# psc0628/NeRF-PRV

Hardware: AMD Instinct MI355X
Metric: ray-samples/s (field evaluations composited; candidate views rendered + scored; scene baseline, field 256^3) (higher is better)
Workload: dtype f16

## Files before the change

### nerf_prv_amd/csrc/prv_kernels.hip

```cpp
#include "prv_kernels.hpp"

#include <algorithm>

#ifndef PRV_ABLATE
#define PRV_ABLATE 0
#endif

namespace prv {


__device__ __forceinline__ void morton16(uint32_t i, uint32_t& x, uint32_t& y) {
  x = (i & 1u) | ((i >> 1) & 2u) | ((i >> 2) & 4u) | ((i >> 3) & 8u);
  y = ((i >> 1) & 1u) | ((i >> 2) & 2u) | ((i >> 3) & 4u) | ((i >> 4) & 8u);
}

constexpr float kNgpDt = 1.7320508075688772f / 1024.0f;

__device__ __forceinline__ uint32_t march_ngp(const FieldDev& fd, const float o[3], const float d[3], float t0, float t1,
                                              uint32_t (*mw)[256], int& k_lo, int& k_hi, int& first_nz, int& last_nz) {
  const float dt = kNgpDt;
  first_nz = 32;
  last_nz = -1;
  k_lo = k_hi = 0;
  float ta = t0, tb = t1;
#pragma unroll
  for (int a = 0; a < 3; a++) {
    const float inv = 1.0f / d[a];
    const float u = (fd.occ_lo[a] - o[a]) * inv, w = (fd.occ_hi[a] - o[a]) * inv;
    ta = fmaxf(ta, fminf(u, w));
    tb = fminf(tb, fmaxf(u, w));
  }
  if (!(tb > ta)) return 0u;
  const float inv_dt = 1024.0f / 1.7320508075688772f;
  const int g_lo = max(0, (int)((ta - t0) * inv_dt) - 2);
  const int g_hi = min(kNgpMaxSteps, (int)((tb - t0) * inv_dt) + 3);
  if (g_lo >= g_hi) return 0u;
  k_lo = g_lo >> 5;
  k_hi = (g_hi + 31) >> 5;
  const bool coarse_ok = fd.occ_coarse != nullptr && 16.0f * dt <= 0.99f * 4.0f / (float)fd.occ_res;
  const int Rc_m1 = (fd.occ_res >> 2) - 1;
  const float fRc = (float)(fd.occ_res >> 2);
  const uint32_t Rc = (uint32_t)(Rc_m1 + 1);
  uint32_t n_live = 0u;
  for (int k = k_lo; k < k_hi; k++) {
    uint32_t w = 0u;
    bool pass = true;
    if (coarse_ok) {
      const float tm = fmaf((float)(32 * k + 16), dt, t0);
      const int cx = min(max((int)(fmaf(tm, d[0], o[0]) * fRc), 0), Rc_m1), cy = min(max((int)(fmaf(tm, d[1], o[1]) * fRc), 0), Rc_m1),
                cz = min(max((int)(fmaf(tm, d[2], o[2]) * fRc), 0), Rc_m1);
      const uint32_t bit = (uint32_t)cx + Rc * ((uint32_t)cy + Rc * (uint32_t)cz);
      pass = (fd.occ_coarse[bit >> 5] >> (bit & 31u)) & 1u;
    }
    if (pass) {
#pragma unroll
      for (int q0 = 0; q0 < 32; q0 += 8) {
        bool occ[8];
#pragma unroll
        for (int q = 0; q < 8; q++) {
          const int i = 32 * k + q0 + q;
          const float t = fmaf((float)i + 0.5f, dt, t0);
          occ[q] = occupied(fd, fmaf(t, d[0], o[0]), fmaf(t, d[1], o[1]), fmaf(t, d[2], o[2])) && t < t1;
        }
#pragma unroll
        for (int q = 0; q < 8; q++) w |= (uint32_t)occ[q] << (q0 + q);
      }
    }
    mw[k][threadIdx.x] = w;
    if (w != 0u) {
      if (first_nz == 32) first_nz = k;
      last_nz = k;
      n_live += (uint32_t)__popc(w);
    }
  }
  return n_live;
}


struct MarchRay {
  float o[3], d[3], t0, t1;
  uint32_t pix;
  bool valid, hit;
};

template <class PT>
__device__ __forceinline__ void march_ray_setup(const PT& P, const float occ_lo[3], const float occ_hi[3], uint32_t tx, uint32_t ty, MarchRay& r) {
  const uint32_t vi = blockIdx.y;
  uint32_t ix, iy, kk;
  if (P.spp_inner_log2 > 0) {
    kk = threadIdx.x & ((1u << P.spp_inner_log2) - 1u);
    morton16(threadIdx.x >> P.spp_inner_log2, ix, iy);
  } else {
    kk = blockIdx.z;
    morton16(threadIdx.x, ix, iy);
  }
  const int px = (int)((tx << P.tile_w_log2) + ix), py = (int)((ty << P.tile_h_log2) + iy);
  r.valid = px < P.W && py < P.H;
  r.pix = ((kk * gridDim.y + (uint32_t)vi) * (uint32_t)P.H + (uint32_t)py) * (uint32_t)P.W + (uint32_t)px;
  r.o[0] = r.o[1] = r.o[2] = 0.f;
  r.d[0] = r.d[1] = 0.f;
  r.d[2] = 1.f;
  r.t0 = r.t1 = 0.f;
  r.hit = false;
  bool maybe = r.valid;
  const CamDev& cam = P.cams[P.view_ids[vi]];
  float ox, oy;
  spp_offset((int)kk, ox, oy);
  if (cam.cull[2] > 0) {
    const int x0 = (int)(tx << P.tile_w_log2), y0 = (int)(ty << P.tile_h_log2);
    if (x0 + (1 << P.tile_w_log2) <= cam.cull[0] || x0 >= cam.cull[2] || y0 + (1 << P.tile_h_log2) <= cam.cull[1] || y0 >= cam.cull[3]) maybe = false;
  }
  if (maybe && !has_lens(cam)) {
    const float far = fmaxf(fmaxf(fabsf(cam.c2w[3] - 0.5f), fabsf(cam.c2w[7] - 0.5f)), fabsf(cam.c2w[11] - 0.5f));
    const float grow = fmaf(far, 1e-5f, 1e-3f);
    const float x = (((float)px + ox) - cam.cx) * __builtin_amdgcn_rcpf(cam.fx);
    const float y = (((float)py + oy) - cam.cy) * __builtin_amdgcn_rcpf(cam.fy);
    float ta = 0.0f, tb = __builtin_inff();
#pragma unroll
    for (int a = 0; a < 3; a++) {
      const float* mrow = cam.c2w + a * 4;
      const float inv = __builtin_amdgcn_rcpf(fmaf(mrow[0], x, fmaf(mrow[1], y, mrow[2])));
      const float u = ((occ_lo[a] - grow) - mrow[3]) * inv, w = ((occ_hi[a] + grow) - mrow[3]) * inv;
      ta = fmaxf(ta, fminf(u, w));
      tb = fminf(tb, fmaxf(u, w));
    }
    maybe = !(tb < ta);
  }
#if PRV_ABLATE & 8
  maybe = r.valid;
#endif
  if (maybe) {
    raygen(cam, px, py, ox, oy, r.o, r.d);
    r.hit = ray_aabb(r.o, r.d, r.t0, r.t1);
  }
}

struct MarchSink {
  void* queue;
  uint4* queue_ext;
  size_t ext_stride;
  uint32_t* queue_count;
  float* out_f32;
  uint32_t* out_u8;
};

template <bool NGP, bool WORDS_READY = false, bool IMAGE = true, class PT, class WordFn>
__device__ __forceinline__ void march_write(const PT& P, const MarchSink& Q, uint4 (*stage)[64 * kRecordWords], const MarchRay& r, bool live,
                                            unsigned long long b, uint32_t base, float dt, uint32_t m[4], int first_nz, int last_nz, WordFn word) {
  const int lane = threadIdx.x & 63;
  if (b != 0ull) {
    uint4* st = stage[threadIdx.x >> 6];
    if (live) {
      const uint32_t prefix = (uint32_t)__popcll(b & ((1ull << lane) - 1ull));
      uint4* rec = st + prefix * kRecordWords;
      uint32_t chunk_info = 1u << 16;
      if constexpr (NGP) {
        const int n_chunks = ((last_nz - first_nz) >> 2) + 1;
        chunk_info = (uint32_t)(32 * first_nz) | ((uint32_t)n_chunks << 16);
        if constexpr (!WORDS_READY) {
#pragma unroll
          for (int q = 0; q < 4; q++) m[q] = word(first_nz + q);
          uint4* ext = Q.queue_ext + (size_t)(base + prefix);
          for (int j = 1; j < ((PRV_ABLATE & 128) ? 1 : n_chunks); j++)
            ext[(size_t)(j - 1) * Q.ext_stride] = make_uint4(word(first_nz + 4 * j), word(first_nz + 4 * j + 1), word(first_nz + 4 * j + 2), word(first_nz + 4 * j + 3));
        }
      }
      rec[0] = make_uint4(__float_as_uint(r.o[0]), __float_as_uint(r.o[1]), __float_as_uint(r.o[2]), __float_as_uint(r.t0));
      rec[1] = make_uint4(__float_as_uint(r.d[0]), __float_as_uint(r.d[1]), __float_as_uint(r.d[2]), __float_as_uint(dt));
      rec[2] = make_uint4(m[0], m[1], m[2], m[3]);
      rec[3] = make_uint4(r.pix, chunk_info, 0u, 0u);
      reinterpret_cast<half8*>(rec)[4] = sh_fragment(0, r.d[0], r.d[1], r.d[2]);
      reinterpret_cast<half8*>(rec)[5] = sh_fragment(1, r.d[0], r.d[1], r.d[2]);
    }
    __builtin_amdgcn_fence(__ATOMIC_RELEASE, "wavefront");
    __builtin_amdgcn_wave_barrier();
    __builtin_amdgcn_fence(__ATOMIC_ACQUIRE, "wavefront");
    uint4* dst = reinterpret_cast<uint4*>(Q.queue) + (size_t)base * kRecordWords;
    const uint32_t n_words = (uint32_t)__popcll(b) * kRecordWords;
    for (uint32_t i = (uint32_t)lane; i < ((PRV_ABLATE & 256) ? 1u : n_words); i += 64u) dst[i] = st[i];
  }
  if constexpr (IMAGE) {
    if (!live && r.valid && !(PRV_ABLATE & 64)) {
      reinterpret_cast<float4*>(Q.out_f32)[r.pix] = make_float4(0.f, 0.f, 0.f, 0.f);
      if (P.last_pass && Q.out_u8) Q.out_u8[r.pix] = quantize_rgba8(0.f, 0.f, 0.f, 0.f, P.bg);
    }
  }
}

__device__ __forceinline__ uint32_t ray_octant(const float o[3], const float d[3], float t, const float lo[3], const float hi[3]) {
  uint32_t oct = 0u;
#pragma unroll
  for (int a = 0; a < 3; a++) oct |= (uint32_t)(fmaf(t, d[a], o[a]) > 0.5f * (lo[a] + hi[a])) << a;
  return oct;
}
__device__ __forceinline__ uint32_t region_reserve(uint32_t* queue_count, uint32_t n_seg, uint32_t seg_cap, uint32_t pref, uint32_t n) {
  for (uint32_t k = 0; k < n_seg; k++) {
    const uint32_t shard = (pref + k) % n_seg;
    uint32_t* c = queue_count + 16u * shard;
    if (k != 0u && __hip_atomic_load(c, __ATOMIC_RELAXED, __HIP_MEMORY_SCOPE_AGENT) >= seg_cap) continue;
    const uint32_t old = atomicAdd(c, n);
    if (old + n <= seg_cap) return shard * seg_cap + old;
    if (old < seg_cap) c[1] = seg_cap - old;
  }
  return 0u;
}

template <class PT>
__device__ __forceinline__ void march_count(const PT& P, uint32_t n_live) {
  uint32_t tot = n_live;
#pragma unroll
  for (int sh = 32; sh >= 1; sh >>= 1) tot += (uint32_t)__shfl_xor((int)tot, sh);
  const uint32_t sshard = (blockIdx.x + gridDim.x * (blockIdx.y + gridDim.y * blockIdx.z)) & 7u;
  if ((threadIdx.x & 63) == 0 && tot) atomicAdd(P.stat + 8u * (1u + sshard), (unsigned long long)tot);
}

template <bool NGP, bool IMAGE = true, class PT, class WordFn>
__device__ __forceinline__ void march_emit(const PT& P, const MarchSink& Q, uint4 (*stage)[64 * kRecordWords], const MarchRay& r, bool live,
                                           uint32_t n_live, float dt, uint32_t m[4], int first_nz, int last_nz, WordFn word) {
  const unsigned long long b = __ballot(live);
  const int lane = threadIdx.x & 63;
  uint32_t base = 0;
  if (b != 0ull) {
    if (lane == (int)__builtin_ctzll(b)) {
      uint32_t i0 = 0u;
      if constexpr (NGP) {
        i0 = 32u * (uint32_t)first_nz + (uint32_t)__builtin_ctz(word(first_nz));
        if (P.spatial_regions != 2) i0 = (i0 + 32u * (uint32_t)last_nz + 31u - (uint32_t)__builtin_clz(word(last_nz))) >> 1;
      } else {
        i0 = m[0] ? (uint32_t)__builtin_ctz(m[0]) : m[1] ? 32u + (uint32_t)__builtin_ctz(m[1]) : m[2] ? 64u + (uint32_t)__builtin_ctz(m[2]) : 96u + (uint32_t)__builtin_ctz(m[3]);
        if (P.spatial_regions != 2) {
          const uint32_t i1 = m[3] ? 127u - (uint32_t)__builtin_clz(m[3]) : m[2] ? 95u - (uint32_t)__builtin_clz(m[2]) : m[1] ? 63u - (uint32_t)__builtin_clz(m[1]) : 31u - (uint32_t)__builtin_clz(m[0]);
          i0 = (i0 + i1) >> 1;
        }
      }
      const uint32_t lin = blockIdx.x + gridDim.x * (blockIdx.y + gridDim.y * blockIdx.z);
      const uint32_t pref = P.spatial_regions ? ray_octant(r.o, r.d, fmaf((float)i0 + 0.5f, dt, r.t0), P.field.occ_lo, P.field.occ_hi) * (uint32_t)P.n_sub + lin % (uint32_t)P.n_sub
                                              : lin;
      base = region_reserve(Q.queue_count, (uint32_t)P.n_seg, P.seg_cap, pref % (uint32_t)P.n_seg, (uint32_t)__popcll(b));
    }
    base = __shfl(base, (int)__builtin_ctzll(b));
  }
  march_write<NGP, false, IMAGE>(P, Q, stage, r, live, b, base, dt, m, first_nz, last_nz, word);
  if (b != 0ull) march_count(P, n_live);
}

template <bool NGP, bool IMAGE>
__device__ __forceinline__ void march_compact_body(MarchParams P) {
  __shared__ uint4 stage[4][64 * kRecordWords];
  __shared__ uint32_t mw[NGP ? 32 : 1][256];
  const uint32_t vi = blockIdx.y;
  uint32_t tx, ty;
  if (P.live_grid) {
    const CamDev& cv = P.cams[P.view_ids[vi]];
    uint32_t tx0 = 0, ty0 = 0, tx1 = P.tiles_x, ty1 = P.tiles_y;
    if (cv.cull[2] > 0) {
      tx0 = (uint32_t)cv.cull[0] >> P.tile_w_log2;
      ty0 = (uint32_t)cv.cull[1] >> P.tile_h_log2;
      tx1 = min(P.tiles_x, ((uint32_t)cv.cull[2] + (1u << P.tile_w_log2) - 1u) >> P.tile_w_log2);
      ty1 = min(P.tiles_y, ((uint32_t)max(cv.cull[3], 0) + (1u << P.tile_h_log2) - 1u) >> P.tile_h_log2);
    }
    const uint32_t w = tx1 > tx0 ? tx1 - tx0 : 0u, h = ty1 > ty0 ? ty1 - ty0 : 0u;
    if (blockIdx.x >= w * h) return;
    ty = ty0 + blockIdx.x / w;
    tx = tx0 + blockIdx.x - (blockIdx.x / w) * w;
  } else {
    ty = blockIdx.x / P.tiles_x;
    tx = blockIdx.x - ty * P.tiles_x;
  }
  MarchRay r;
  march_ray_setup(P, P.field.occ_lo, P.field.occ_hi, tx, ty, r);
  const float* o = r.o;
  const float* d = r.d;
  const float t0 = r.t0, t1 = r.t1;
  float dt = 0.f;
  uint32_t m[4] = {0, 0, 0, 0};
  uint32_t n_live = 0u;
  int k_lo = 0, k_hi = 0, first_nz = 32, last_nz = -1;
  bool live = false;
#if PRV_ABLATE & 32
  r.hit = false;
#endif
  if (r.hit) {
#if PRV_ABLATE & 16
    live = (t0 + t1 + d[0] + o[1]) == 1.0e30f;
#else
    if constexpr (NGP) {
      dt = kNgpDt;
      n_live = march_ngp(P.field, o, d, t0, t1, mw, k_lo, k_hi, first_nz, last_nz);
      live = first_nz < 32;
    } else {
      dt = (t1 - t0) / (float)P.S;
      const bool coarse_ok = P.field.occ_coarse != nullptr && 1.5f * dt <= 0.99f * 4.0f / (float)P.field.occ_res;
      int g_lo = 0, g_hi = P.S;
      {
        float ta = t0, tb = t1;
#pragma unroll
        for (int a = 0; a < 3; a++) {
          const float inv = 1.0f / d[a];
          const float u = (P.field.occ_lo[a] - o[a]) * inv, w = (P.field.occ_hi[a] - o[a]) * inv;
          ta = fmaxf(ta, fminf(u, w));
          tb = fminf(tb, fmaxf(u, w));
        }
        if (!(tb > ta)) {
          g_hi = 0;
        } else if (dt > 0.0f) {
          const float inv_dt = __builtin_amdgcn_rcpf(dt);
          g_lo = max(0, (int)((ta - t0) * inv_dt) - 2) & ~3;
          g_hi = min(P.S, (int)((tb - t0) * inv_dt) + 3);
        }
      }
      const int Rc_m1 = (P.field.occ_res >> 2) - 1;
      const float fRc = (float)(P.field.occ_res >> 2);
      const float ocx = o[0] * fRc, ocy = o[1] * fRc, ocz = o[2] * fRc, dcx = d[0] * fRc, dcy = d[1] * fRc, dcz = d[2] * fRc;
      const uint32_t Rc = (uint32_t)(Rc_m1 + 1);
#pragma unroll
      for (int k = 0; k < 4; k++) {
        uint32_t w = 0u;
        const int lo = max(g_lo, 32 * k), hi = min(g_hi, 32 * k + 32);
        if (lo < hi) {
          uint32_t pass = 0xffu;
          if (coarse_ok) {
            pass = 0u;
#pragma unroll
            for (int j = 0; j < 8; j++) {
              const int g = 32 * k + 4 * j;
// ... 146 lines not shown
    for (int e = 0; e < E; e++) {
      first_any = min(first_any, first_nz[e]);
      last_any = max(last_any, last_nz[e]);
    }
    const unsigned long long b_any = __ballot(first_any < 32);
    uint32_t pref = blockIdx.x + gridDim.x * (blockIdx.y + gridDim.y * blockIdx.z);
    if (P.spatial_regions && b_any != 0ull) {
      const uint32_t oct = ray_octant(o, d, fmaf((float)(16 * (min(first_any, 31) + last_any)) + 16.0f, dt, t0), P.occ_lo, P.occ_hi);
      pref = (uint32_t)__shfl((int)oct, (int)__builtin_ctzll(b_any)) * (uint32_t)P.n_sub + pref % (uint32_t)P.n_sub;
    }
    const uint32_t shard = pref % (uint32_t)P.n_seg;
    uint32_t* qc = nullptr;
    uint32_t mine = 0u, tot = 0u;
#pragma unroll
    for (int e = 0; e < E; e++) {
      b[e] = __ballot(first_nz[e] < 32);
      if (lane == e) {
        qc = P.mem[e].queue_count;
        mine = (uint32_t)__popcll(b[e]);
      }
      tot += n_live[e];
    }
    uint32_t got = 0u;
    if (mine) got = region_reserve(qc, (uint32_t)P.n_seg, P.seg_cap, shard, mine);
#pragma unroll
    for (int e = 0; e < E; e++) base[e] = __shfl(got, e);
    march_count(P, tot);
  }
  uint32_t m[E][4];
#pragma unroll
  for (int e = 0; e < E; e++)
#pragma unroll
    for (int q = 0; q < 4; q++) m[e][q] = 0u;
  {
    int k2_lo = 32, k2_hi = -1;
#pragma unroll
    for (int e = 0; e < E; e++) {
      k2_lo = min(k2_lo, first_nz[e]);
      k2_hi = max(k2_hi, last_nz[e]);
    }
    uint32_t acc[E][4];
#pragma unroll
    for (int e = 0; e < E; e++)
#pragma unroll
      for (int q = 0; q < 4; q++) acc[e][q] = 0u;
    for (int k = k2_lo; k <= k2_hi; k++) {
      uint32_t w[E];
      bool behind = false;
#pragma unroll
      for (int e = 0; e < E; e++) behind = behind || (k - first_nz[e] >= kWin && k <= last_nz[e]);
      if (!((passmask >> k) & 1u)) {
#pragma unroll
        for (int e = 0; e < E; e++) w[e] = 0u;
      } else if (behind) {
        fine_word(k, w);
      } else {
#pragma unroll
        for (int e = 0; e < E; e++) {
          const int j = k - first_nz[e];
          w[e] = (j >= 0 && k <= last_nz[e]) ? mw[e][j][threadIdx.x] : 0u;
        }
      }
#pragma unroll
      for (int e = 0; e < E; e++) {
        const int j = k - first_nz[e];
        if (j < 0 || k > last_nz[e]) continue;
        const int q = j & 3;
        if (j < 4) {
#pragma unroll
          for (int u = 0; u < 4; u++)
            if (q == u) m[e][u] = w[e];
        } else {
#pragma unroll
          for (int u = 0; u < 4; u++)
            if (q == u) acc[e][u] = w[e];
          if ((q == 3 || k == last_nz[e]) && !(PRV_ABLATE & 128)) {
            const uint32_t slot = base[e] + (uint32_t)__popcll(b[e] & ((1ull << lane) - 1ull));
            P.mem[e].queue_ext[(size_t)((j >> 2) - 1) * ext_stride + slot] = make_uint4(acc[e][0], acc[e][1], acc[e][2], acc[e][3]);
#pragma unroll
            for (int u = 0; u < 4; u++) acc[e][u] = 0u;
          }
        }
      }
    }
  }
#pragma unroll
  for (int e = 0; e < E; e++) {
    const MarchSink Q{P.mem[e].queue, P.mem[e].queue_ext, ext_stride, P.mem[e].queue_count, P.mem[e].out_f32, P.mem[e].out_u8};
    march_write<true, true>(P, Q, stage, r, first_nz[e] < 32, b[e], base[e], dt, m[e], first_nz[e], last_nz[e], [](int) { return 0u; });
  }
}

__global__ __launch_bounds__(256) void occ_interleave_kernel(OccInterleaveParams P) {
  const uint32_t c = blockIdx.x * 256u + threadIdx.x;
  if (c >= P.n_cells) return;
  uint32_t v = 0u;
  for (int e = 0; e < P.n_members; e++) v |= ((P.bits[e][c >> 5] >> (c & 31u)) & 1u) << e;
  P.out[c] = (uint8_t)v;
}


__device__ __forceinline__ void clock_stamp_begin(unsigned long long* stat) {
  if (blockIdx.x == 0 && threadIdx.x == 0) {
    stat[4] = __builtin_readcyclecounter();
    stat[5] = __builtin_amdgcn_s_memrealtime();
  }
}
__device__ __forceinline__ void clock_stamp_end(unsigned long long* stat) {
  if (blockIdx.x == 0 && threadIdx.x == 0) {
    atomicAdd(stat + 2, __builtin_readcyclecounter() - stat[4]);
    atomicAdd(stat + 3, __builtin_amdgcn_s_memrealtime() - stat[5]);
  }
}

__device__ __forceinline__ int lane_id() { return (int)(threadIdx.x & 63u); }

__device__ __forceinline__ float entropy_add(float p, float H) { return p >= 1.17549435e-38f ? fmaf(p, -__builtin_amdgcn_logf(p), H) : H; }

template <int F, int NDENSE, bool NGP, bool CACHE, int MODE>
__device__ __forceinline__ void render_queue64_body(RenderParams P, const RenderPlanesParams* X) {
  constexpr bool FOOT = MODE == kRenderFootprint, SURF = MODE == kRenderSurface;
  constexpr bool DEPTH = MODE == kRenderDepth || FOOT, ENTROPY = MODE == kRenderEntropy || FOOT || SURF;
  constexpr bool DSTATE = DEPTH || SURF;
  constexpr int kDWord = ENTROPY ? 4 : 6;
  constexpr int kMoveWords = (ENTROPY ? 4 : 6) + (DSTATE ? 1 : 0);
  constexpr int kFrags = ENTROPY ? 8 : kNumFrags;
  __shared__ half8 wl[kFrags * 64];
  __shared__ uint32_t mv[4][32][kMoveWords];
  constexpr uint32_t kPoolCap = 192;
  __shared__ uint32_t pool[kPoolCap][kMoveWords];
  __shared__ uint32_t pool_n, pool_lock;
  for (int i = threadIdx.x; i < kFrags * 64; i += 256) wl[i] = P.field.frags64[i];
  if (threadIdx.x == 0) {
    pool_n = 0u;
    pool_lock = 0u;
  }
  __syncthreads();
  auto pool_acquire = [&]() {
    if (lane_id() == 0)
      while (atomicCAS(&pool_lock, 0u, 1u) != 0u) __builtin_amdgcn_s_sleep(2);
    __builtin_amdgcn_fence(__ATOMIC_ACQUIRE, "workgroup");
    __builtin_amdgcn_wave_barrier();
  };
  auto pool_release = [&]() {
    __builtin_amdgcn_fence(__ATOMIC_RELEASE, "workgroup");
    __builtin_amdgcn_wave_barrier();
    if (lane_id() == 0) atomicExch(&pool_lock, 0u);
  };
  const LevelDev* __restrict__ lvl = P.field.levels;
  const HashConsts hc = {P.field.hash_my_b, P.field.hash_mz_b, P.field.hash_m_b, (uint32_t)P.field.wide_offsets};

  const int lane = threadIdx.x & 63, r = lane & 31, g = lane >> 5;

  bool active = false;
  uint32_t pix = 0, rec_i = 0;
  float o[3] = {0, 0, 0}, d[3] = {0, 0, 1}, t0 = 0.f, dt = 0.f;
  uint32_t cur = 0, m1 = 0, m2 = 0, m3 = 0, base = 0;
  float T = 1.f, cr = 0.f, cg = 0.f, cb = 0.f;
  float D = 0.f;
  float Hs = 0.f;
  half8 shA = {0, 0, 0, 0, 0, 0, 0, 0}, shB = {0, 0, 0, 0, 0, 0, 0, 0};
  bool drained = false;
  unsigned long long n_eval = 0ull, n_rounds = 0ull;
  constexpr int kCached = CACHE ? 32 / F - NDENSE : 1;
  CornerCache<F> cc[kCached];
#pragma unroll
  for (int j = 0; j < kCached; j++) cc[j].key = ~0u;
  clock_stamp_begin(P.stat_evaluated);
  uint32_t q_cur = 0, q_end = 0;
  const uint32_t n_seg = (uint32_t)P.n_segments;
  const uint32_t n_sub = (uint32_t)max(P.n_sub, 1);
  uint32_t seg = n_seg > 1u ? (((uint32_t)__builtin_amdgcn_s_getreg((3 << 11) | 20) & 7u) % (n_seg / n_sub)) * n_sub + (blockIdx.x * 4u + (threadIdx.x >> 6)) % n_sub : 0u;
  uint32_t seg_tried = 0;
  const uint4* __restrict__ queue = reinterpret_cast<const uint4*>(P.queue);

  auto take_ray = [&](uint32_t ri, uint32_t next) {
    const uint4* rec = queue + (size_t)ri * kRecordWords;
    const uint4 q0 = rec[0], q1 = rec[1], q3 = rec[3];
    uint4 mk = rec[2];
    o[0] = __uint_as_float(q0.x); o[1] = __uint_as_float(q0.y); o[2] = __uint_as_float(q0.z);
    t0 = __uint_as_float(q0.w);
    d[0] = __uint_as_float(q1.x); d[1] = __uint_as_float(q1.y); d[2] = __uint_as_float(q1.z);
    dt = __uint_as_float(q1.w);
    pix = q3.x;
    rec_i = ri;
    base = 0u;
    if constexpr (NGP) {
      const uint32_t base0 = q3.y & 0xffffu;
      base = base0;
      if (next >= base0 + 128u) {
        const uint32_t j = (next - base0) >> 7;
        mk = P.queue_ext[(size_t)(j - 1u) * ((size_t)P.seg_cap * (size_t)P.n_segments) + (size_t)ri];
        base = base0 + 128u * j;
      }
    }
    cur = mk.x; m1 = mk.y; m2 = mk.z; m3 = mk.w;
    while (base + 32u <= next) {
      cur = m1; m1 = m2; m2 = m3; m3 = 0u;
      base += 32u;
    }
    if (next > base) cur &= ~0u << (next & 31u);
    while (cur == 0u && (m1 | m2 | m3) != 0u) {
      cur = m1; m1 = m2; m2 = m3; m3 = 0u;
      base += 32u;
    }
    active = true;
  };
  auto next_chunk = [&]() -> bool {
    const uint32_t info = queue[(size_t)rec_i * kRecordWords + 3].y;
    const uint32_t base0 = info & 0xffffu, n_chunks = info >> 16;
    for (uint32_t j = ((base - base0) >> 7) + 1u; j < n_chunks; j++) {
      const uint4 mk = P.queue_ext[(size_t)(j - 1u) * ((size_t)P.seg_cap * (size_t)P.n_segments) + (size_t)rec_i];
      if ((mk.x | mk.y | mk.z | mk.w) == 0u) continue;
      cur = mk.x; m1 = mk.y; m2 = mk.z; m3 = mk.w;
      base = base0 + 128u * j;
      while (cur == 0u) {
        cur = m1; m1 = m2; m2 = m3; m3 = 0u;
        base += 32u;
      }
      return true;
    }
    return false;
  };

  for (;;) {
    const bool relocate = (n_rounds & 6ull) == 0ull;
    if (relocate && !drained && P.merge_max > 0) {
      const unsigned long long act0 = __ballot(active);
      const uint32_t aA = (uint32_t)act0, aB = (uint32_t)(act0 >> 32);
      const uint32_t nA = (uint32_t)__popc(aA), nB = (uint32_t)__popc(aB);
      int src = -1;
      if (nA != 0u && nB != 0u) {
        if (nA <= (uint32_t)P.merge_max && nA <= 32u - nB) src = 0;
        else if (nB <= (uint32_t)P.merge_max && nB <= 32u - nA) src = 1;
      }
      if (src >= 0) {
        const uint32_t a_src = src == 0 ? aA : aB, a_dst = src == 0 ? aB : aA, n_src = src == 0 ? nA : nB;
        const uint32_t below = (1u << r) - 1u;
        uint32_t(*slot)[kMoveWords] = mv[threadIdx.x >> 6];
        if (g == src && active) {
          uint32_t* e = slot[__popc(a_src & below)];
          e[0] = rec_i;
          e[1] = base + (uint32_t)__builtin_ctz(cur);
          e[2] = __float_as_uint(T);
          if constexpr (ENTROPY) {
            e[3] = __float_as_uint(Hs);
          } else {
            e[3] = __float_as_uint(cr);
            e[4] = __float_as_uint(cg);
            e[5] = __float_as_uint(cb);
          }
          if constexpr (DSTATE) e[kDWord] = __float_as_uint(D);
          active = false;
        }
        __builtin_amdgcn_fence(__ATOMIC_RELEASE, "wavefront");
        __builtin_amdgcn_wave_barrier();
        __builtin_amdgcn_fence(__ATOMIC_ACQUIRE, "wavefront");
        const uint32_t kth = (uint32_t)__popc(~a_dst & below);
        if (!((a_dst >> r) & 1u) && kth < n_src) {
          const uint32_t* e = slot[kth];
          const uint32_t ri = e[0];
          if constexpr (!ENTROPY) {
            const half8 sh = reinterpret_cast<const half8*>(queue + (size_t)ri * kRecordWords)[4 + g];
            if (src == 0) shB = sh;
            else shA = sh;
          }
          if (g != src) {
            T = __uint_as_float(e[2]);
            if constexpr (ENTROPY) {
              Hs = __uint_as_float(e[3]);
            } else {
              cr = __uint_as_float(e[3]); cg = __uint_as_float(e[4]); cb = __uint_as_float(e[5]);
            }
            if constexpr (DSTATE) D = __uint_as_float(e[kDWord]);
            take_ray(ri, e[1]);
          }
        }
        __builtin_amdgcn_wave_barrier();
      }
    }
    if (P.pool_on && (relocate || drained)) {
      const unsigned long long act1 = __ballot(active);
      const uint32_t below = (1u << r) - 1u;
      const uint32_t in_pool = *(volatile uint32_t*)&pool_n;
#pragma unroll
      for (int grp = 0; grp < 2; grp++) {
        const uint32_t a_g = grp == 0 ? (uint32_t)act1 : (uint32_t)(act1 >> 32), n_g = (uint32_t)__popc(a_g);
        if (!drained && n_g != 0u && n_g <= (uint32_t)P.merge_max && in_pool + n_g <= kPoolCap) {
          pool_acquire();
          const uint32_t at = *(volatile uint32_t*)&pool_n;
          const bool fits = at + n_g <= kPoolCap;
          if (fits && g == grp && active) {
            uint32_t* e = pool[at + (uint32_t)__popc(a_g & below)];
            e[0] = rec_i;
            e[1] = base + (uint32_t)__builtin_ctz(cur);
            e[2] = __float_as_uint(T);
            if constexpr (ENTROPY) {
              e[3] = __float_as_uint(Hs);
            } else {
              e[3] = __float_as_uint(cr);
              e[4] = __float_as_uint(cg);
              e[5] = __float_as_uint(cb);
            }
            if constexpr (DSTATE) e[kDWord] = __float_as_uint(D);
            active = false;
          }
          if (fits && lane == 0) *(volatile uint32_t*)&pool_n = at + n_g;
          pool_release();
        }
      }
      const unsigned long long act2 = __ballot(active);
#pragma unroll
      for (int grp = 0; grp < 2; grp++) {
        const uint32_t a_g = grp == 0 ? (uint32_t)act2 : (uint32_t)(act2 >> 32);
        const uint32_t n_idle = 32u - (uint32_t)__popc(a_g);
        if (n_idle == 0u || (a_g == 0u && !drained) || *(volatile uint32_t*)&pool_n == 0u) continue;
        pool_acquire();
        const uint32_t have = *(volatile uint32_t*)&pool_n;
        const uint32_t take = min(have, n_idle), from = have - take;
        const uint32_t kth = (uint32_t)__popc(~a_g & below);
        uint32_t ent[kMoveWords] = {};
        const bool mine = !((a_g >> r) & 1u) && kth < take;
        if (mine) {
#pragma unroll
          for (int q = 0; q < kMoveWords; q++) ent[q] = pool[from + kth][q];
        }
        if (lane == 0) *(volatile uint32_t*)&pool_n = from;
        pool_release();
        if (mine) {
          if constexpr (!ENTROPY) {
            const half8 sh = reinterpret_cast<const half8*>(queue + (size_t)ent[0] * kRecordWords)[4 + g];
            if (grp == 0) shA = sh;
            else shB = sh;
          }
          if (g == grp) {
            T = __uint_as_float(ent[2]);
            if constexpr (ENTROPY) {
              Hs = __uint_as_float(ent[3]);
            } else {
              cr = __uint_as_float(ent[3]); cg = __uint_as_float(ent[4]); cb = __uint_as_float(ent[5]);
            }
            if constexpr (DSTATE) D = __uint_as_float(ent[kDWord]);
            take_ray(ent[0], ent[1]);
          }
        }
      }
    }
    const unsigned long long idle = __ballot(!active);
    const bool needA = (uint32_t)idle == 0xffffffffu, needB = (uint32_t)(idle >> 32) == 0xffffffffu;
    if (!drained && (needA || needB)) {
#pragma unroll
      for (int grp = 0; grp < 2; grp++) {
        if (!(grp == 0 ? needA : needB)) continue;
        while (q_cur == q_end && !drained) {
          uint32_t claim = 0;
          if (lane == 0) claim = atomicAdd(P.queue_head + 16u * seg, kClaim);
          claim = __builtin_amdgcn_readfirstlane(claim);
          const uint32_t s_lo = seg * P.seg_cap, s_cnt = min(P.queue_count[16u * seg], P.seg_cap) - P.queue_count[16u * seg + 1u];
          if (claim < s_cnt) {
            q_cur = s_lo + claim;
            q_end = min(q_cur + kClaim, s_lo + s_cnt);
          } else if (++seg_tried >= n_seg) {
            drained = true;
          } else {
            seg = seg + 1u == n_seg ? 0u : seg + 1u;
          }
        }
        const uint32_t avail = min(32u, q_end - q_cur);
        if ((uint32_t)r < avail) {
          if constexpr (!ENTROPY) {
            const half8 sh = reinterpret_cast<const half8*>(queue + (size_t)(q_cur + (uint32_t)r) * kRecordWords)[4 + g];
            if (grp == 0) shA = sh;
            else shB = sh;
          }
          if (g == grp) {
            T = 1.f; cr = 0.f; cg = 0.f; cb = 0.f;
            if constexpr (DSTATE) D = 0.f;
            if constexpr (ENTROPY) Hs = 0.f;
            take_ray(q_cur + (uint32_t)r, 0u);
          }
        }
        q_cur += avail;
      }
    }
    const unsigned long long act = __ballot(active);
    if (act == 0ull) {
      if (drained && (!P.pool_on || *(volatile uint32_t*)&pool_n == 0u)) break;
      continue;
    }
    n_eval += (unsigned long long)__popcll(act);
    n_rounds += 2ull;

    half8 f[4];
#pragma unroll
    for (int s = 0; s < 4; s++) asm volatile("" : "=v"(f[s]));
    bool last = false;
    float ts = 0.f;
    if (active) {
      const uint32_t i = base + (uint32_t)__builtin_ctz(cur);
      cur &= cur - 1u;
      if (cur == 0u) {
        last = (m1 | m2 | m3) == 0u;
        while (cur == 0u && !last) {
          cur = m1; m1 = m2; m2 = m3; m3 = 0u;
          base += 32u;
        }
        if constexpr (NGP) {
          if (last) last = !next_chunk();
        }
      }
      const float t = fmaf((float)i + 0.5f, dt, t0);
      if constexpr (DSTATE) ts = t;
      encode_sample<F, NDENSE, CACHE>(P.field.table, lvl, hc, fmaf(t, d[0], o[0]), fmaf(t, d[1], o[1]), fmaf(t, d[2], o[2]), f, cc);
    }
    swap_halves(f[0], f[1]);
    swap_halves(f[2], f[3]);
    const half8 fA[2] = {f[0], f[2]}, fB[2] = {f[1], f[3]};
    MlpOut2 mo;
    if constexpr (ENTROPY) mlp_density2(wl, lane, fA, fB, mo.densA, mo.densB);
    else mo = mlp_forward2(wl, lane, fA, fB, shA, shB);
    const float dens = g ? mo.densB[8] : mo.densA[0];
    float lr = 0.f, lg = 0.f, lb = 0.f;
    if constexpr (!ENTROPY) {
      lr = g ? mo.rgbB[8] : mo.rgbA[0];
      lg = g ? mo.rgbB[9] : mo.rgbA[1];
      lb = g ? mo.rgbB[10] : mo.rgbA[2];
    }

    bool done = false;
    if (active) {
      const float sigma = fast_exp(dens + P.field.density_bias);
      const float alpha = 1.0f - fast_exp(-(sigma * dt));
      const float wgt = alpha * T;
      if constexpr (ENTROPY) {
        Hs = entropy_add(wgt, Hs);
      } else {
        cr = fmaf(wgt, fast_sigmoid(lr), cr);
        cg = fmaf(wgt, fast_sigmoid(lg), cg);
        cb = fmaf(wgt, fast_sigmoid(lb), cb);
      }
      if constexpr (DEPTH) D = fmaf(wgt, ts, D);
      T = T * (1.0f - alpha);
      if constexpr (SURF) {
        if (D == 0.f && T <= X->T_cross) D = ts;
      }
      done = last || T < P.min_T;
    }
    if (done) {
      if constexpr (!ENTROPY) {
        const float4 v = make_float4(cr, cg, cb, 1.0f - T);
        reinterpret_cast<float4*>(P.out_f32)[pix] = v;
        if (P.last_pass && P.out_u8) P.out_u8[pix] = quantize_rgba8(v.x, v.y, v.z, v.w, P.bg);
      }
      if constexpr (ENTROPY) {
        X->out_entropy[pix] = entropy_add(T, Hs);
        X->out_alpha[pix] = 1.0f - T;
      }
      if constexpr (DSTATE) {
        const CamDev& cam = X->cams[X->view_ids[(pix / X->npix) % X->nb]];
        const float fx = cam.c2w[2], fy = cam.c2w[6], fz = cam.c2w[10];
        const float inv = 1.0f / sqrtf(fmaf(fx, fx, fmaf(fy, fy, fz * fz)));
        X->out_depth[pix] = D * (fmaf(d[0], fx, fmaf(d[1], fy, d[2] * fz)) * inv);
        if constexpr (SURF) X->out_hit[pix] = D > 0.f ? 1.0f : 0.0f;
      }
      active = false;
    }
  }
  if (lane == 0 && n_eval) {
    atomicAdd(P.stat_evaluated, n_eval);
    atomicAdd(P.stat_evaluated + 1, n_rounds);
  }
  clock_stamp_end(P.stat_evaluated);
}

template <int F, int NDENSE, bool NGP, bool CACHE = false>
__global__ __launch_bounds__(256)
__attribute__((amdgpu_waves_per_eu(CACHE ? 2 : NDENSE == 0 ? 1 : 3)))
void render_queue64_kernel(RenderParams P) {
  render_queue64_body<F, NDENSE, NGP, CACHE, kRenderColour>(P, nullptr);
}

template <int F, int NDENSE, bool NGP, int MODE>
__global__ __launch_bounds__(256)
__attribute__((amdgpu_waves_per_eu(NDENSE == 0 ? 1 : MODE == kRenderSurface && F == 4 && !NGP ? 4 : 3)))
void render_planes_kernel(RenderPlanesParams P) {
  render_queue64_body<F, NDENSE, NGP, false, MODE>(P.r, &P);
}

__device__ __forceinline__ int32_t first_hit_dda(const FieldDev& fd, const float o[3], const float d[3], float max_range) {
  float t0, t1;
  int32_t result = -1;
  if (ray_aabb(o, d, t0, t1)) {
    if (t1 > max_range) t1 = max_range;
    if (t1 > t0) {
      const int R = fd.occ_res;
      const float fR = (float)R;
      const float ts = t0 + 1e-6f;
      int c[3], step[3];
      float tmax[3], tdelta[3];
#pragma unroll
      for (int a = 0; a < 3; a++) {
        const float p = clamp01(fmaf(ts, d[a], o[a])) * fR;
        c[a] = min((int)p, R - 1);
        if (d[a] > 0.f) {
          step[a] = 1;
          tmax[a] = (((float)(c[a] + 1)) / fR - o[a]) / d[a];
          tdelta[a] = 1.0f / (fR * d[a]);
        } else if (d[a] < 0.f) {
          step[a] = -1;
          tmax[a] = (((float)c[a]) / fR - o[a]) / d[a];
          tdelta[a] = -1.0f / (fR * d[a]);
        } else {
          step[a] = 0;
          tmax[a] = __builtin_inff();
          tdelta[a] = __builtin_inff();
        }
      }
      for (;;) {
        const uint32_t bit = (uint32_t)c[0] + (uint32_t)R * ((uint32_t)c[1] + (uint32_t)R * (uint32_t)c[2]);
        if ((fd.occ[bit >> 5] >> (bit & 31)) & 1u) {
          result = (int32_t)bit;
          break;
        }
        const int a = tmax[0] < tmax[1] ? (tmax[0] < tmax[2] ? 0 : 2) : (tmax[1] < tmax[2] ? 1 : 2);
        const float tm = a == 0 ? tmax[0] : (a == 1 ? tmax[1] : tmax[2]);
        if (tm > t1) break;
        if (a == 0) { c[0] += step[0]; tmax[0] += tdelta[0]; if (c[0] < 0 || c[0] >= R) break; }
        else if (a == 1) { c[1] += step[1]; tmax[1] += tdelta[1]; if (c[1] < 0 || c[1] >= R) break; }
        else { c[2] += step[2]; tmax[2] += tdelta[2]; if (c[2] < 0 || c[2] >= R) break; }
      }
    }
  }
  return result;
}

__global__ __launch_bounds__(256) void first_hit_kernel(FieldDev fd, const CamDev* __restrict__ cams, int W, int H,
                                                        float max_range, int32_t* __restrict__ out) {
  const int i = blockIdx.x * 256 + threadIdx.x;
  if (i >= W * H) return;
  const int v = blockIdx.y;
  const int px = i % W, py = i / W;
  float o[3], d[3], t0, t1;
  raygen(cams[v], px, py, 0.5f, 0.5f, o, d);
  (void)t0;
  (void)t1;
  const int32_t result = first_hit_dda(fd, o, d, max_range);
  out[(size_t)v * W * H + i] = result;
}

__global__ __launch_bounds__(256) void precept_kernel(FieldDev fd, const float* __restrict__ voxels, int n, PreceptPose pose,
                                                      Rs2Intr in, float max_range, int32_t* __restrict__ out) {
  const int i = blockIdx.x * 256 + threadIdx.x;
  if (i >= n) return;
  const float origin[3] = {(float)pose.c2w[3], (float)pose.c2w[7], (float)pose.c2w[11]};
  double v[3];
#pragma unroll
  for (int r = 0; r < 3; r++)
    v[r] = pose.w2c[r * 4] * (double)voxels[i * 3] + pose.w2c[r * 4 + 1] * (double)voxels[i * 3 + 1] +
           pose.w2c[r * 4 + 2] * (double)voxels[i * 3 + 2] + pose.w2c[r * 4 + 3];
  const float point_3d[3] = {(float)v[0], (float)v[1], (float)v[2]};
  float pixel[2];
  rs2_project(pixel, in, point_3d);
  int32_t result = -1;
  if (!(pixel[0] < 0 || pixel[0] > (float)in.width || pixel[1] < 0 || pixel[1] > (float)in.height)) {
    const float ipx[2] = {(float)(int)pixel[0], (float)(int)pixel[1]};
    float pt[3], d[3];
    rs2_deproject(pt, in, ipx, 1.0f);
#pragma unroll
    for (int r = 0; r < 3; r++) {
      const float e = (float)(pose.c2w[r * 4] * (double)pt[0] + pose.c2w[r * 4 + 1] * (double)pt[1] +
                              pose.c2w[r * 4 + 2] * (double)pt[2] + pose.c2w[r * 4 + 3]);
      d[r] = e - origin[r];
    }
    const float n2 = fmaf(d[0], d[0], fmaf(d[1], d[1], d[2] * d[2]));
    const float inv = 1.0f / sqrtf(n2);
#pragma unroll
    for (int r = 0; r < 3; r++) d[r] = d[r] * inv;
    result = first_hit_dda(fd, origin, d, max_range);
  }
  out[i] = result;
}

__global__ __launch_bounds__(256) void spp_reduce_kernel(const float4* __restrict__ stage, size_t n, int spp, float inv_spp,
                                                         float b0, float b1, float b2, float b3,
                                                         float4* __restrict__ out, uint32_t* __restrict__ out_u8) {
  const float bg[4] = {b0, b1, b2, b3};
  for (size_t i = (size_t)blockIdx.x * 256 + threadIdx.x; i < n; i += (size_t)gridDim.x * 256) {
    float4 a = stage[i];
    for (int k = 1; k < spp; k++) {
      const float4 v = stage[(size_t)k * n + i];
      a.x = a.x + v.x; a.y = a.y + v.y; a.z = a.z + v.z; a.w = a.w + v.w;
    }
    a.x *= inv_spp; a.y *= inv_spp; a.z *= inv_spp; a.w *= inv_spp;
    out[i] = a;
    if (out_u8) out_u8[i] = quantize_rgba8(a.x, a.y, a.z, a.w, bg);
  }
}

__global__ __launch_bounds__(256) void spp_reduce_depth_kernel(const float* __restrict__ stage, size_t n, int spp, float inv_spp,
                                                               float* __restrict__ out) {
  for (size_t i = (size_t)blockIdx.x * 256 + threadIdx.x; i < n; i += (size_t)gridDim.x * 256) {
    float a = stage[i];
    for (int k = 1; k < spp; k++) a = a + stage[(size_t)k * n + i];
    out[i] = a * inv_spp;
  }
}


__global__ __launch_bounds__(256) void quantize_kernel(const float4* __restrict__ in, size_t n,
                                                       float b0, float b1, float b2, float b3,
                                                       uint32_t* __restrict__ out) {
  const float bg[4] = {b0, b1, b2, b3};
  for (size_t i = (size_t)blockIdx.x * 256 + threadIdx.x; i < n; i += (size_t)gridDim.x * 256) {
    float4 v = in[i];
    out[i] = quantize_rgba8(v.x, v.y, v.z, v.w, bg);
  }
}


// ... 644 lines not shown
```

### nerf_prv_amd/csrc/prv_kernels.hpp

```cpp
#pragma once
#include "../../include/prv.h"
#include "prv_device.hpp"
#include <type_traits>

namespace prv {

constexpr size_t kRecordBytes = 96;
constexpr int kRecordWords = 6;
constexpr uint32_t kClaim = 64;
constexpr int kMaxSamples = 128;
constexpr int kNgpMaxSteps = PRV_NGP_MAX_STEPS;
constexpr int kExtChunks = kNgpMaxSteps / 128 - 1;
constexpr size_t kExtBytes = (size_t)kExtChunks * 16;

struct MarchParams {
  FieldDev field;
  const CamDev* cams;
  const int* view_ids;
  int W, H, S;
  uint32_t tiles_x, tiles_y;
  int tile_w_log2, tile_h_log2;
  int spp_inner_log2;
  int live_grid;
  uint32_t live_tiles_max;
  int step_mode;
  void* queue;
  uint4* queue_ext;
  unsigned long long* stat;
  uint32_t* queue_count;
  int n_seg;
  uint32_t seg_cap;
  int spatial_regions;
  int n_sub;
  float* out_f32;
  uint32_t* out_u8;
  int last_pass;
  float bg[4];
};

struct MarchMember {
  void* queue;
  uint4* queue_ext;
  uint32_t* queue_count;
  float* out_f32;
  uint32_t* out_u8;
};
struct MarchMultiParams {
  const uint8_t* occ_bytes;
  const uint8_t* occ_coarse_bytes;
  int occ_res;
  float occ_lo[3], occ_hi[3];
  const CamDev* cams;
  const int* view_ids;
  int W, H;
  uint32_t tiles_x, tiles_y;
  int tile_w_log2, tile_h_log2, spp_inner_log2;
  unsigned long long* stat;
  int n_seg;
  uint32_t seg_cap;
  int spatial_regions, n_sub;
  int last_pass;
  float bg[4];
  int n_members;
  MarchMember mem[PRV_MAX_MODELS];
};
struct OccInterleaveParams {
  const uint32_t* bits[PRV_MAX_MODELS];
  int n_members;
  uint32_t n_cells;
  uint8_t* out;
};
bool march_multi_supported(int n_members);
hipError_t launch_march_multi(const MarchMultiParams& P, int n_views, int n_spp, hipStream_t s);
hipError_t launch_occ_interleave(const OccInterleaveParams& P, hipStream_t s);

struct RenderParams {
  FieldDev field;
  const void* queue;
  const uint4* queue_ext;
  int step_mode;
  const uint32_t* queue_count;
  uint32_t* queue_head;
  int n_segments;
  int n_sub;
  uint32_t seg_cap;
  unsigned long long* stat_evaluated;
  float* out_f32;
  uint32_t* out_u8;
  float min_T;
  int last_pass;
  int merge_max;
  int pool_on;
  int cell_cache;
  float bg[4];
};

enum : int { kRenderColour = 0, kRenderDepth = 1, kRenderEntropy = 2, kRenderFootprint = 3, kRenderSurface = 4 };

struct RenderPlanesParams {
  RenderParams r;
  float* out_depth;
  const CamDev* cams;
  const int* view_ids;
  uint32_t npix;
  uint32_t nb;
  float* out_entropy;
  float* out_alpha;
  float T_cross;
  float* out_hit;
};

struct EnsembleParams {
  const uint32_t* imgs[PRV_MAX_MODELS];
  int E;
  int view0;
  size_t pixels_per_view;
  double* partial;
};

struct PsnrParams {
  const float* rgba;
  const float* gt;
  const CamDev* cams;
  int W;
  size_t pixels_per_view;
  float bg[4];
  double* partial;
};

struct RepackLevel {
  uint32_t canon_off, phys_off, n, res, sx, hashed;
};
hipError_t launch_repack_level(const uint16_t* canon, uint16_t* phys, const RepackLevel& L, int F, hipStream_t s);

hipError_t launch_march(const MarchParams& P, int n_views, int n_spp, hipStream_t s);
hipError_t launch_spp_reduce(const float* stage, size_t n_pixels, int spp, const float bg[4], float* out, uint32_t* out_u8,
                             hipStream_t s);
hipError_t launch_render(const RenderParams& P, int n_blocks, hipStream_t s);
hipError_t launch_render_planes(const RenderPlanesParams& P, int mode, int n_blocks, hipStream_t s);
hipError_t launch_spp_reduce_depth(const float* stage, size_t n_pixels, int spp, float* out, hipStream_t s);
hipError_t launch_score_entropy(const float* entropy, const float* alpha, size_t npix, int n_views, int n_blocks, double* partial,
                                hipStream_t s);
inline int render_instance_dense_levels(const FieldDev& fd) {
  const int n = fd.n_dense_levels;
  if (!fd.hash_shared) return 0;
  if (fd.n_features == 4) return n == 5 ? 5 : n == 3 ? 3 : 0;
  return n == 10 ? 10 : n == 6 ? 6 : 0;
}
template <class Fn>
void with_field_instance(const FieldDev& fd, Fn&& fn) {
  using std::integral_constant;
  const int nd = render_instance_dense_levels(fd);
  if (fd.n_features == 4) {
    if (nd == 5) fn(integral_constant<int, 4>{}, integral_constant<int, 5>{});
    else if (nd == 3) fn(integral_constant<int, 4>{}, integral_constant<int, 3>{});
    else fn(integral_constant<int, 4>{}, integral_constant<int, 0>{});
  } else {
    if (nd == 10) fn(integral_constant<int, 2>{}, integral_constant<int, 10>{});
    else if (nd == 6) fn(integral_constant<int, 2>{}, integral_constant<int, 6>{});
    else fn(integral_constant<int, 2>{}, integral_constant<int, 0>{});
  }
// ... 27 lines not shown
```

Measured before the change: 24.33 billion.

## Shrink ray queue records, recompute SH rows, track wave activity as scalar mask

Ray queue records drop from 96 to 64 bytes because the two precomputed spherical-harmonics half8 fragments are no longer stored. The render loop recomputes them from the direction word it already loads. The per-lane active flag becomes a wave-uniform 64-bit mask that is updated incrementally, which removes repeated ballots and lets the pool be skipped when it is not needed. Bitmask advance gets a fast path for the common case. This trades queue write/read bandwidth and vector ballots for extra SH arithmetic at each ray refill.

```diff
diff --git a/nerf_prv_amd/csrc/prv_kernels.hip b/nerf_prv_amd/csrc/prv_kernels.hip
--- a/nerf_prv_amd/csrc/prv_kernels.hip
+++ b/nerf_prv_amd/csrc/prv_kernels.hip
@@ -169,8 +169,6 @@
       rec[1] = make_uint4(__float_as_uint(r.d[0]), __float_as_uint(r.d[1]), __float_as_uint(r.d[2]), __float_as_uint(dt));
       rec[2] = make_uint4(m[0], m[1], m[2], m[3]);
       rec[3] = make_uint4(r.pix, chunk_info, 0u, 0u);
-      reinterpret_cast<half8*>(rec)[4] = sh_fragment(0, r.d[0], r.d[1], r.d[2]);
-      reinterpret_cast<half8*>(rec)[5] = sh_fragment(1, r.d[0], r.d[1], r.d[2]);
     }
     __builtin_amdgcn_fence(__ATOMIC_RELEASE, "wavefront");
     __builtin_amdgcn_wave_barrier();
@@ -623,7 +621,9 @@
 
   const int lane = threadIdx.x & 63, r = lane & 31, g = lane >> 5;
 
-  bool active = false;
+  unsigned long long act = 0ull;
+  auto active = [&]() -> bool { return __builtin_amdgcn_inverse_ballot_w64(act); };
+  auto pool_count = [&]() -> uint32_t { return (uint32_t)__builtin_amdgcn_readfirstlane((int)*(volatile uint32_t*)&pool_n); };
   uint32_t pix = 0, rec_i = 0;
   float o[3] = {0, 0, 0}, d[3] = {0, 0, 1}, t0 = 0.f, dt = 0.f;
   uint32_t cur = 0, m1 = 0, m2 = 0, m3 = 0, base = 0;
@@ -641,13 +641,14 @@
   uint32_t q_cur = 0, q_end = 0;
   const uint32_t n_seg = (uint32_t)P.n_segments;
   const uint32_t n_sub = (uint32_t)max(P.n_sub, 1);
-  uint32_t seg = n_seg > 1u ? (((uint32_t)__builtin_amdgcn_s_getreg((3 << 11) | 20) & 7u) % (n_seg / n_sub)) * n_sub + (blockIdx.x * 4u + (threadIdx.x >> 6)) % n_sub : 0u;
+  const uint32_t wave_in_block = (uint32_t)__builtin_amdgcn_readfirstlane((int)(threadIdx.x >> 6));
+  uint32_t seg = n_seg > 1u ? (((uint32_t)__builtin_amdgcn_s_getreg((3 << 11) | 20) & 7u) % (n_seg / n_sub)) * n_sub + (blockIdx.x * 4u + wave_in_block) % n_sub : 0u;
   uint32_t seg_tried = 0;
   const uint4* __restrict__ queue = reinterpret_cast<const uint4*>(P.queue);
 
-  auto take_ray = [&](uint32_t ri, uint32_t next) {
+  auto take_ray = [&](uint32_t ri, uint32_t next, const uint4 q1) {
     const uint4* rec = queue + (size_t)ri * kRecordWords;
-    const uint4 q0 = rec[0], q1 = rec[1], q3 = rec[3];
+    const uint4 q0 = rec[0], q3 = rec[3];
     uint4 mk = rec[2];
     o[0] = __uint_as_float(q0.x); o[1] = __uint_as_float(q0.y); o[2] = __uint_as_float(q0.z);
     t0 = __uint_as_float(q0.w);
@@ -675,8 +676,8 @@
       cur = m1; m1 = m2; m2 = m3; m3 = 0u;
       base += 32u;
     }
-    active = true;
   };
+  auto sh_rows = [&](const uint4 q1) { return sh_fragment(g, __uint_as_float(q1.x), __uint_as_float(q1.y), __uint_as_float(q1.z)); };
   auto next_chunk = [&]() -> bool {
     const uint32_t info = queue[(size_t)rec_i * kRecordWords + 3].y;
     const uint32_t base0 = info & 0xffffu, n_chunks = info >> 16;
@@ -697,8 +698,7 @@
   for (;;) {
     const bool relocate = (n_rounds & 6ull) == 0ull;
     if (relocate && !drained && P.merge_max > 0) {
-      const unsigned long long act0 = __ballot(active);
-      const uint32_t aA = (uint32_t)act0, aB = (uint32_t)(act0 >> 32);
+      const uint32_t aA = (uint32_t)act, aB = (uint32_t)(act >> 32);
       const uint32_t nA = (uint32_t)__popc(aA), nB = (uint32_t)__popc(aB);
       int src = -1;
       if (nA != 0u && nB != 0u) {
@@ -709,7 +709,7 @@
         const uint32_t a_src = src == 0 ? aA : aB, a_dst = src == 0 ? aB : aA, n_src = src == 0 ? nA : nB;
         const uint32_t below = (1u << r) - 1u;
         uint32_t(*slot)[kMoveWords] = mv[threadIdx.x >> 6];
-        if (g == src && active) {
+        if (g == src && active()) {
           uint32_t* e = slot[__popc(a_src & below)];
           e[0] = rec_i;
           e[1] = base + (uint32_t)__builtin_ctz(cur);
@@ -722,17 +722,18 @@
             e[5] = __float_as_uint(cb);
           }
           if constexpr (DSTATE) e[kDWord] = __float_as_uint(D);
-          active = false;
         }
         __builtin_amdgcn_fence(__ATOMIC_RELEASE, "wavefront");
         __builtin_amdgcn_wave_barrier();
         __builtin_amdgcn_fence(__ATOMIC_ACQUIRE, "wavefront");
         const uint32_t kth = (uint32_t)__popc(~a_dst & below);
-        if (!((a_dst >> r) & 1u) && kth < n_src) {
+        const bool mine = !((a_dst >> r) & 1u) && kth < n_src;
+        if (mine) {
           const uint32_t* e = slot[kth];
           const uint32_t ri = e[0];
+          const uint4 q1 = queue[(size_t)ri * kRecordWords + 1];
           if constexpr (!ENTROPY) {
-            const half8 sh = reinterpret_cast<const half8*>(queue + (size_t)ri * kRecordWords)[4 + g];
+            const half8 sh = sh_rows(q1);
             if (src == 0) shB = sh;
             else shA = sh;
           }
@@ -744,24 +745,32 @@
               cr = __uint_as_float(e[3]); cg = __uint_as_float(e[4]); cb = __uint_as_float(e[5]);
             }
             if constexpr (DSTATE) D = __uint_as_float(e[kDWord]);
-            take_ray(ri, e[1]);
+            take_ray(ri, e[1], q1);
           }
         }
+        act = (src == 0 ? act & ~0xffffffffull : act & 0xffffffffull) | __ballot(mine && g != src);
         __builtin_amdgcn_wave_barrier();
       }
     }
+    bool pool_look = false;
     if (P.pool_on && (relocate || drained)) {
-      const unsigned long long act1 = __ballot(active);
+#pragma unroll
+      for (int grp = 0; grp < 2; grp++) {
+        const uint32_t a_g = grp == 0 ? (uint32_t)act : (uint32_t)(act >> 32), n_g = (uint32_t)__popc(a_g);
+        pool_look = pool_look || (!drained && n_g != 0u && n_g <= (uint32_t)P.merge_max) || (a_g != 0xffffffffu && (a_g != 0u || drained));
+      }
+    }
+    if (pool_look) {
       const uint32_t below = (1u << r) - 1u;
-      const uint32_t in_pool = *(volatile uint32_t*)&pool_n;
+      const uint32_t in_pool = pool_count();
 #pragma unroll
       for (int grp = 0; grp < 2; grp++) {
-        const uint32_t a_g = grp == 0 ? (uint32_t)act1 : (uint32_t)(act1 >> 32), n_g = (uint32_t)__popc(a_g);
+        const uint32_t a_g = grp == 0 ? (uint32_t)act : (uint32_t)(act >> 32), n_g = (uint32_t)__popc(a_g);
         if (!drained && n_g != 0u && n_g <= (uint32_t)P.merge_max && in_pool + n_g <= kPoolCap) {
           pool_acquire();
-          const uint32_t at = *(volatile uint32_t*)&pool_n;
+          const uint32_t at = pool_count();
           const bool fits = at + n_g <= kPoolCap;
-          if (fits && g == grp && active) {
+          if (fits && g == grp && active()) {
             uint32_t* e = pool[at + (uint32_t)__popc(a_g & below)];
             e[0] = rec_i;
             e[1] = base + (uint32_t)__builtin_ctz(cur);
@@ -774,20 +783,19 @@
               e[5] = __float_as_uint(cb);
             }
             if constexpr (DSTATE) e[kDWord] = __float_as_uint(D);
-            active = false;
           }
           if (fits && lane == 0) *(volatile uint32_t*)&pool_n = at + n_g;
           pool_release();
-        }
-      }
-      const unsigned long long act2 = __ballot(active);
+          if (fits) act &= grp == 0 ? ~0xffffffffull : 0xffffffffull;
+        }
+      }
 #pragma unroll
       for (int grp = 0; grp < 2; grp++) {
-        const uint32_t a_g = grp == 0 ? (uint32_t)act2 : (uint32_t)(act2 >> 32);
+        const uint32_t a_g = grp == 0 ? (uint32_t)act : (uint32_t)(act >> 32);
         const uint32_t n_idle = 32u - (uint32_t)__popc(a_g);
-        if (n_idle == 0u || (a_g == 0u && !drained) || *(volatile uint32_t*)&pool_n == 0u) continue;
+        if (n_idle == 0u || (a_g == 0u && !drained) || pool_count() == 0u) continue;
         pool_acquire();
-        const uint32_t have = *(volatile uint32_t*)&pool_n;
+        const uint32_t have = pool_count();
         const uint32_t take = min(have, n_idle), from = have - take;
         const uint32_t kth = (uint32_t)__popc(~a_g & below);
         uint32_t ent[kMoveWords] = {};
@@ -799,8 +807,9 @@
         if (lane == 0) *(volatile uint32_t*)&pool_n = from;
         pool_release();
         if (mine) {
+          const uint4 q1 = queue[(size_t)ent[0] * kRecordWords + 1];
           if constexpr (!ENTROPY) {
-            const half8 sh = reinterpret_cast<const half8*>(queue + (size_t)ent[0] * kRecordWords)[4 + g];
+            const half8 sh = sh_rows(q1);
             if (grp == 0) shA = sh;
             else shB = sh;
           }
@@ -812,13 +821,13 @@
               cr = __uint_as_float(ent[3]); cg = __uint_as_float(ent[4]); cb = __uint_as_float(ent[5]);
             }
             if constexpr (DSTATE) D = __uint_as_float(ent[kDWord]);
-            take_ray(ent[0], ent[1]);
+            take_ray(ent[0], ent[1], q1);
           }
         }
-      }
-    }
-    const unsigned long long idle = __ballot(!active);
-    const bool needA = (uint32_t)idle == 0xffffffffu, needB = (uint32_t)(idle >> 32) == 0xffffffffu;
+        act |= __ballot(mine && g == grp);
+      }
+    }
+    const bool needA = (uint32_t)act == 0u, needB = (uint32_t)(act >> 32) == 0u;
     if (!drained && (needA || needB)) {
 #pragma unroll
       for (int grp = 0; grp < 2; grp++) {
@@ -838,9 +847,11 @@
           }
         }
         const uint32_t avail = min(32u, q_end - q_cur);
-        if ((uint32_t)r < avail) {
+        const bool fill = (uint32_t)r < avail;
+        if (fill) {
+          const uint4 q1 = queue[(size_t)(q_cur + (uint32_t)r) * kRecordWords + 1];
           if constexpr (!ENTROPY) {
-            const half8 sh = reinterpret_cast<const half8*>(queue + (size_t)(q_cur + (uint32_t)r) * kRecordWords)[4 + g];
+            const half8 sh = sh_rows(q1);
             if (grp == 0) shA = sh;
             else shB = sh;
           }
@@ -848,15 +859,15 @@
             T = 1.f; cr = 0.f; cg = 0.f; cb = 0.f;
             if constexpr (DSTATE) D = 0.f;
             if constexpr (ENTROPY) Hs = 0.f;
-            take_ray(q_cur + (uint32_t)r, 0u);
+            take_ray(q_cur + (uint32_t)r, 0u, q1);
           }
         }
+        act |= __ballot(fill && g == grp);
         q_cur += avail;
       }
     }
-    const unsigned long long act = __ballot(active);
     if (act == 0ull) {
-      if (drained && (!P.pool_on || *(volatile uint32_t*)&pool_n == 0u)) break;
+      if (drained && (!P.pool_on || pool_count() == 0u)) break;
       continue;
     }
     n_eval += (unsigned long long)__popcll(act);
@@ -867,17 +878,23 @@
     for (int s = 0; s < 4; s++) asm volatile("" : "=v"(f[s]));
     bool last = false;
     float ts = 0.f;
-    if (active) {
+    const bool on = active();
+    if (on) {
       const uint32_t i = base + (uint32_t)__builtin_ctz(cur);
       cur &= cur - 1u;
       if (cur == 0u) {
-        last = (m1 | m2 | m3) == 0u;
-        while (cur == 0u && !last) {
+        if (m1 != 0u) {
           cur = m1; m1 = m2; m2 = m3; m3 = 0u;
           base += 32u;
-        }
-        if constexpr (NGP) {
-          if (last) last = !next_chunk();
+        } else {
+          last = (m2 | m3) == 0u;
+          while (cur == 0u && !last) {
+            cur = m1; m1 = m2; m2 = m3; m3 = 0u;
+            base += 32u;
+          }
+          if constexpr (NGP) {
+            if (last) last = !next_chunk();
+          }
         }
       }
       const float t = fmaf((float)i + 0.5f, dt, t0);
@@ -898,8 +915,7 @@
       lb = g ? mo.rgbB[10] : mo.rgbA[2];
     }
 
-    bool done = false;
-    if (active) {
+    if (on) {
       const float sigma = fast_exp(dens + P.field.density_bias);
       const float alpha = 1.0f - fast_exp(-(sigma * dt));
       const float wgt = alpha * T;
@@ -915,8 +931,8 @@
       if constexpr (SURF) {
         if (D == 0.f && T <= X->T_cross) D = ts;
       }
-      done = last || T < P.min_T;
-    }
+    }
+    const bool done = on && (last || T < P.min_T);
     if (done) {
       if constexpr (!ENTROPY) {
         const float4 v = make_float4(cr, cg, cb, 1.0f - T);
@@ -934,8 +950,8 @@
         X->out_depth[pix] = D * (fmaf(d[0], fx, fmaf(d[1], fy, d[2] * fz)) * inv);
         if constexpr (SURF) X->out_hit[pix] = D > 0.f ? 1.0f : 0.0f;
       }
-      active = false;
-    }
+    }
+    act &= ~__ballot(done);
   }
   if (lane == 0 && n_eval) {
     atomicAdd(P.stat_evaluated, n_eval);
diff --git a/nerf_prv_amd/csrc/prv_kernels.hpp b/nerf_prv_amd/csrc/prv_kernels.hpp
--- a/nerf_prv_amd/csrc/prv_kernels.hpp
+++ b/nerf_prv_amd/csrc/prv_kernels.hpp
@@ -5,8 +5,8 @@
 
 namespace prv {
 
-constexpr size_t kRecordBytes = 96;
-constexpr int kRecordWords = 6;
+constexpr int kRecordWords = 4;
+constexpr size_t kRecordBytes = 16 * (size_t)kRecordWords;
 constexpr uint32_t kClaim = 64;
 constexpr int kMaxSamples = 128;
 constexpr int kNgpMaxSteps = PRV_NGP_MAX_STEPS;
```

Result: no change. 24.34 billion, median of 2 (+0.0%).
